# mumianyuxin/M3DSSD

Measured on AMD Instinct MI355X. Metric: images/sec at 1280x384 bs=8, 1/2/4/8 MI355X; 3D-box Linf vs ref, higher is better.
Workload: dtype f32; 1 GPU; BASELINE.json configs[1]: full M3d_inference_align (DLA-34 + DCNv2 align + ANAB) forward + decode + top-3000 + NMS, bs=8/GPU, 1280x384, fp32, random-init synthetic weights and frames; per_gpu_batch=8, global_batch=8, parallelism=dp1 (batch sharded, 1 all-gather of [B,40,14] detections)

## Files before the change

include/m3dssd_hip.h:

```cpp
#ifndef M3DSSD_HIP_H
#define M3DSSD_HIP_H

#include <stdint.h>

#ifdef __cplusplus
extern "C" {
#endif

typedef void *m3d_stream_t;

enum {
    M3D_OK = 0,
    M3D_E_ARG = -1,
    M3D_E_HIP = -2,
    M3D_E_WORKSPACE = -3
};

const char *m3d_last_error(void);
#define M3D_ABI_VERSION 5
int m3d_abi_version(void);
const char *m3d_source_hashes(void);

typedef struct m3d_conv_desc {
    const float *in;
// ... 263 lines not shown
    M3D_RPN_STAT_IOU_ACC = 7,
    M3D_RPN_STAT_ACC_FG = 8,
    M3D_RPN_STAT_ACC_BG = 9,
    M3D_RPN_STAT_N_FG = 10,
    M3D_RPN_STAT_N_BG = 11,
    M3D_RPN_STAT_FG_NUM = 12,
    M3D_RPN_STAT_BG_NUM = 13,
    M3D_RPN_STAT_N_ACTIVE = 14,
    M3D_RPN_STAT_FG_WEIGHT = 15,
    M3D_RPN_STAT_COUNT = 16
};
long long m3d_rpn_loss_workspace_bytes(int B, long long R);
int m3d_rpn_targets(const double *anchors, int A, int H, int W, const double *conf, int n_conf, const double *gt_table, int B,
                    int Gmax, const float *cls, const float *prob, int C, short *labels, short *gt_index, float *targets,
                    float *scores, void *workspace, long long workspace_bytes, m3d_stream_t stream);
int m3d_rpn_loss(const double *anchors, int A, int H, int W, const double *conf, int n_conf, const double *gt_table, int B,
                 int Gmax, const float *cls, const float *bbox_2d, const float *bbox_3d, int C, const short *labels,
                 const float *targets, const float *scores, unsigned char *sampled, float *grad_cls, float *grad_bbox_2d,
                 float *grad_bbox_3d, float *loss, double *stats, void *workspace, long long workspace_bytes,
                 m3d_stream_t stream);

enum {
    M3D_RPN_SMP_STAT_BAD_LABELS = 16,
    M3D_RPN_SMP_STAT_COUNT = 17
};
int m3d_rpn_precompute_targets(const double *anchors, int A, int H, int W, const double *conf, int n_conf,
                               const double *gt_table, int B, int Gmax, short *labels, short *gt_index, float *bbox_2d_tar,
                               float *bbox_3d_tar, int *any_val, void *workspace, long long workspace_bytes,
                               m3d_stream_t stream);
int m3d_rpn_loss_smp(const double *anchors, int A, int H, int W, const double *conf, int n_conf, int B, const void *labels_in,
                     int label_bytes, const float *bbox_2d_tar, const float *bbox_3d_tar, const int *any_val, const float *cls,
                     const float *prob, const float *bbox_2d, const float *bbox_3d, int C, short *labels, float *targets,
                     float *scores, unsigned char *sampled, float *grad_cls, float *grad_bbox_2d, float *grad_bbox_3d,
                     float *loss, double *stats, void *workspace, long long workspace_bytes, m3d_stream_t stream);

#define M3D_RPN_TARGET_STATS_COLS 23
long long m3d_rpn_target_stats_workspace_bytes(int B, long long R);
int m3d_rpn_target_stats(const double *anchors, int A, int H, int W, const double *conf, int n_conf, const double *gt_table, int B,
                         int Gmax, const double *center, double *out, void *workspace, long long workspace_bytes,
                         m3d_stream_t stream);

int m3d_pack_conv_weight(const float *w, float *packed, int Cout, int Cout_pad, int Cin, int Cin_pad, int kh,
                         int kw, m3d_stream_t stream);
int m3d_nchw_to_nhwc(const float *in, float *out, int N, int C, int H, int W, int out_cs, m3d_stream_t stream);
int m3d_nhwc_to_nchw(const float *in, int in_cs, float *out, int N, int C, int H, int W, m3d_stream_t stream);

int m3d_stem_conv7x7(const float *img_nchw, const float *wgt , const float *scale,
                     const float *shift, float *out, int out_cs, int N, int H, int W, m3d_stream_t stream);
int m3d_preprocess_u8(const unsigned char *frames_bgr, int N, int img_h, int img_w, const float *mean3, const float *stds3,
                      float *out_nchw, int H, int W, m3d_stream_t stream);
int m3d_stem_conv7x7_u8(const unsigned char *frames_bgr, int img_h, int img_w, const float *mean3, const float *stds3,
                        const float *wgt, const float *scale, const float *shift, float *out, int out_cs, int N, int H, int W,
                        m3d_stream_t stream);
#define M3D_AUGMENT_PARAMS 14
int m3d_augment_u8(const unsigned char *frames_bgr, int N, int hmax, int wmax, const double *params, int param_stride,
                   const float *mean3, const float *stds3, float *out_nchw, int H, int W, m3d_stream_t stream);
int m3d_conv3x3_c16(const float *in, int in_cs, const float *wgt, const float *scale, const float *shift, float *out,
                    int out_cs, int N, int H, int W, m3d_stream_t stream);
int m3d_conv3x3_c16_wino(const float *in, int in_cs, const float *U, const float *scale, const float *shift, float *out,
                         int out_cs, int N, int H, int W, m3d_stream_t stream);
int m3d_maxpool2x2(const float *in, int in_cs, float *out, int out_cs, int N, int H, int W, int C,
                   m3d_stream_t stream);
int m3d_upsample2x_add(const float *in, int in_cs, const float *wgt, const float *skip, int skip_cs,
                       float *out, int out_cs, int N, int H, int W, int C, m3d_stream_t stream);

int m3d_anchor_select(const float *cls_planar, int B, int A, int num_classes, int HW, int *sel_idx,
                      float *sel_prob, float *fg_all, m3d_stream_t stream);
int m3d_anchor_select_keys(const float *cls_planar, int B, int A, int HW, int *sel_idx, float *sel_prob,
                           unsigned int *score_bits, m3d_stream_t stream);
int m3d_fg_top1(const float *prob, int B, int A, int HW, int *idx, float *val, m3d_stream_t stream);
int m3d_align_offsets(int mode, const int *sel_idx, const float *sel_prob, float thresh, const float *table,
                      const float *bbox_x, const float *bbox_y, const float *anchor_wh, float mean_x,
                      float std_x, float mean_y, float std_y, float *offmask, int om_cs, int B, int A, int HW,
                      int kk, long long box_img_stride, m3d_stream_t stream);
int m3d_align_offsets_gated(const int *sel_idx, const float *sel_prob, float thresh, const float *bbox_x, const float *bbox_y,
                            const float *anchor_wh, float mean_x, float std_x, float mean_y, float std_y,
                            const unsigned char *need, float *offmask, int om_cs, int B, int A, int HW,
                            long long box_img_stride, m3d_stream_t stream);

int m3d_anab_pool_partial(const float *kv, int kv_cs, const float *s, int s_cs, const int *items, int n_items,
                          const int *bin_scale, int n_bins, float *partial, int max_slots, int B, int H, int W,
                          int C, m3d_stream_t stream);
int m3d_anab_pool_finish(const float *partial, const int *bin_slots, const float *bin_inv_area, int n_bins,
                         int max_slots, int Ck, int Cv, float *khat, int keys_pad, int ck_pad, float *vhatT,
                         int B, int frag, m3d_stream_t stream);
long long m3d_anab_pool_nested_scratch_bytes(int B, int C);
int m3d_anab_pool_nested(const float *kv, int kv_cs, const float *s, int s_cs, int B, int H, int W, int Ck, int Cv,
                         float *scratch, float *khat, int keys_pad, int ck_pad, float *vhatT, int frag, m3d_stream_t stream);
int m3d_anab_pool_nested_bf16(const void *kv, int kv_cs, const float *s, int s_cs, int B, int H, int W, int Ck, int Cv,
                              float *scratch, float *khat, int keys_pad, int ck_pad, float *vhatT, int frag, m3d_stream_t stream);
int m3d_anab_pool_nested_bf16_ex(const void *kv, int kv_cs, const float *s, int s_cs, int B, int H, int W, int Ck, int Cv,
                                 float *scratch, float *khat, int keys_pad, int ck_pad, float *vhatT, int frag,
                                 void *khat16, void *vhat16, m3d_stream_t stream);
int m3d_anab_attend_f32(const float *q, int q_cs, const float *khat, int k_cs, const float *vhatT, int B, int HW, int Ck,
                        int keys, int keys_pad, int Cv, const float *res, int res_cs, int res_mode, const float *scale,
                        const float *shift, int act, float *out, int out_cs, m3d_stream_t stream);
int m3d_anab_attend_f32_rows(const float *q, int q_cs, const float *khat, int k_cs, const float *vhatT, int B, int HW, int Ck,
                             int keys, int keys_pad, int Cv, const float *res, int res_cs, int res_mode, const float *scale,
                             const float *shift, int act, float *out, int out_cs, const int *rows, const int *n_rows,
                             m3d_stream_t stream);
long long m3d_anab_attention_workspace_bytes(int B, int H, int W, int Ck, int Cv, int backward);
int m3d_anab_attention_forward(const float *q, const float *k, const float *v, const float *g, float *out, int B, int H, int W, int Ck,
                               int Cv, int q_cs, int k_cs, int v_cs, int g_cs, int out_cs, void *workspace, long long workspace_bytes,
                               m3d_stream_t stream);
int m3d_anab_attention_backward(const float *q, const float *k, const float *v, const float *g, const float *grad_out, float *grad_q,
                                float *grad_k, float *grad_v, float *grad_g, int B, int H, int W, int Ck, int Cv, int q_cs, int k_cs,
// ... 83 lines not shown
```

m3dssd_amd/_hip.py:

```python
import ctypes
import os
import subprocess

_HERE = os.path.dirname(os.path.abspath(__file__))
CSRC = os.path.join(_HERE, "csrc")
SO_PATH = os.environ.get("M3D_HIP_LIB") or os.path.join(CSRC, "build", "libm3dssd_hip.so")
HEADER = os.path.join(os.path.dirname(_HERE), "include", "m3dssd_hip.h")

c_int, c_float, c_ll, c_void_p = ctypes.c_int, ctypes.c_float, ctypes.c_longlong, ctypes.c_void_p


class ConvDesc(ctypes.Structure):
    _fields_ = [
        ("inp", c_void_p), ("in_cs", c_int),
        ("N", c_int), ("H", c_int), ("W", c_int), ("Cin", c_int),
        ("wgt", c_void_p), ("wgt_img_stride", c_ll),
        ("Cout", c_int), ("Cout_pad", c_int),
        ("kh", c_int), ("kw", c_int), ("stride", c_int), ("pad", c_int), ("dil", c_int),
        ("Ho", c_int), ("Wo", c_int),
        ("out", c_void_p), ("out_cs", c_int), ("out_nchw", c_int), ("out_img_stride", c_ll),
        ("scale", c_void_p), ("shift", c_void_p),
        ("res", c_void_p), ("res_cs", c_int), ("res_mode", c_int),
        ("act", c_int), ("sigmoid_from", c_int),
        ("dcn_offmask", c_void_p), ("dcn_om_cs", c_int),
# ... 113 lines not shown
    "m3d_head_mlp_forward_batched": (c_int, [ctypes.POINTER(MlpDesc), c_int, P]),
    "m3d_head_mlp_forward_rows": (c_int, [ctypes.POINTER(MlpDesc), c_int, P, P, ctypes.c_uint, P]),
    "m3d_wino_conv3x3_forward": (c_int, [ctypes.POINTER(ConvDesc), P]),
    "m3d_wino_conv3x3_forward_ex": (c_int, [ctypes.POINTER(ConvDesc), c_int, P]),
    "m3d_wino_conv3x3_splitk_plan": (c_int, [ctypes.POINTER(ConvDesc), ctypes.POINTER(c_int), ctypes.POINTER(c_ll)]),
    "m3d_wino_conv3x3_variant": (c_int, [ctypes.POINTER(ConvDesc)]),
    "m3d_wino44_applicable": (c_int, [ctypes.POINTER(ConvDesc)]),
    "m3d_wino44_conv3x3_forward": (c_int, [ctypes.POINTER(ConvDesc), P]),
    "m3d_wino44_conv3x3_forward_ex": (c_int, [ctypes.POINTER(ConvDesc), c_int, P]),
    "m3d_wino44_kpair": (c_int, [ctypes.POINTER(ConvDesc)]),
    "m3d_wino44_conv3x3_forward_touch": (c_int, [ctypes.POINTER(ConvDesc), c_int, P, c_ll, P]),
    "m3d_cache_touch": (c_int, [P, c_ll, P]),
    "m3d_upload_indirect": (c_int, [P, P, c_ll, P]),
    "m3d_wino44_splitk_plan": (c_int, [ctypes.POINTER(ConvDesc), ctypes.POINTER(c_int), ctypes.POINTER(c_ll)]),
    "m3d_conv_wave_applicable": (c_int, [ctypes.POINTER(ConvDesc)]),
    "m3d_conv_wave_splitk_plan": (c_int, [ctypes.POINTER(ConvDesc), ctypes.POINTER(c_int), ctypes.POINTER(c_ll)]),
    "m3d_conv_wave_forward": (c_int, [ctypes.POINTER(ConvDesc), P]),
    "m3d_conv_wave_forward_wgsplit": (c_int, [ctypes.POINTER(ConvDesc), P]),
    "m3d_conv_wave_wgsplit_width": (c_int, [ctypes.POINTER(ConvDesc), ctypes.POINTER(c_int), ctypes.POINTER(c_int)]),
    "m3d_conv2d_tile": (c_int, [ctypes.POINTER(ConvDesc)] + [ctypes.POINTER(c_int)] * 4),
    "m3d_conv2d_splitk_plan": (c_int, [ctypes.POINTER(ConvDesc), ctypes.POINTER(c_int), ctypes.POINTER(c_ll)]),
    "m3d_dcn_v2_workspace_bytes": (c_ll, [c_int] * 10),
    "m3d_dcn_v2_workspace_bytes_grouped": (c_ll, [c_int] * 11),
    "m3d_dcn_v2_forward": (c_int, [P] * 6 + [c_int] * 14 + [P, c_ll, P]),
    "m3d_dcn_v2_backward_workspace_bytes": (c_ll, [c_int] * 11),
    "m3d_dcn_v2_backward": (c_int, [P] * 10 + [c_int] * 14 + [P, c_ll, P]),
    "m3d_dcn_v2_workspace_bytes_bf16": (c_ll, [c_int] * 11),
    "m3d_dcn_v2_forward_bf16": (c_int, [P, P, P, P, c_int, P, c_int, P] + [c_int] * 14 + [P, c_ll, P]),
    "m3d_dcn_v2_backward_workspace_bytes_bf16": (c_ll, [c_int] * 11),
    "m3d_dcn_v2_backward_bf16": (c_int, [P, P, P, c_int, P, c_int, P] + [P] * 5 + [c_int] * 14 + [P, c_ll, P]),
    "m3d_dcn_v2_psroi_pooling_workspace_bytes": (c_ll, [c_int] * 10),
    "m3d_dcn_v2_psroi_pooling_forward": (c_int, [P] * 5 + [c_int] * 8 + [c_float] + [c_int] * 5 + [c_float, P, c_ll, P]),
    "m3d_dcn_v2_psroi_pooling_backward": (c_int, [P] * 6 + [c_int] * 8 + [c_float] + [c_int] * 5 + [c_float, P, c_ll, P]),
    "m3d_rpn_loss_workspace_bytes": (c_ll, [c_int, c_ll]),
    "m3d_rpn_targets": (c_int, [P, c_int, c_int, c_int, P, c_int, P, c_int, c_int, P, P, c_int, P, P, P, P, P, c_ll, P]),
    "m3d_rpn_loss": (c_int, [P, c_int, c_int, c_int, P, c_int, P, c_int, c_int, P, P, P, c_int, P, P, P, P, P, P, P, P, P, P, c_ll, P]),
    "m3d_rpn_precompute_targets": (c_int, [P, c_int, c_int, c_int, P, c_int, P, c_int, c_int, P, P, P, P, P, P, c_ll, P]),
    "m3d_rpn_loss_smp": (c_int, [P, c_int, c_int, c_int, P, c_int, c_int, P, c_int, P, P, P, P, P, P, P, c_int] + [P] * 10 + [c_ll, P]),
    "m3d_rpn_target_stats_workspace_bytes": (c_ll, [c_int, c_ll]),
    "m3d_rpn_target_stats": (c_int, [P, c_int, c_int, c_int, P, c_int, P, c_int, c_int, P, P, P, c_ll, P]),
    "m3d_pack_conv_weight": (c_int, [P, P] + [c_int] * 6 + [P]),
    "m3d_nchw_to_nhwc": (c_int, [P, P] + [c_int] * 5 + [P]),
    "m3d_nhwc_to_nchw": (c_int, [P, c_int, P] + [c_int] * 4 + [P]),
    "m3d_stem_conv7x7": (c_int, [P, P, P, P, P] + [c_int] * 4 + [P]),
    "m3d_refine_3d": (c_int, [P, P, c_int, c_int, P, P, ctypes.c_double, c_int, ctypes.c_double, ctypes.c_double, P, P]),
    "m3d_refine_3d_ex": (c_int, [P, P, c_int, c_int, P, P, P, P, ctypes.c_double, c_int, ctypes.c_double, ctypes.c_double, P, P]),
    "m3d_refine_3d_host": (c_int, [P, P, c_int, c_int, P, P, P, P, ctypes.c_double, c_int, ctypes.c_double, ctypes.c_double, P]),
    "m3d_preprocess_u8": (c_int, [P, c_int, c_int, c_int, ctypes.POINTER(ctypes.c_float), ctypes.POINTER(ctypes.c_float), P, c_int,
                                  c_int, P]),
    "m3d_augment_u8": (c_int, [P, c_int, c_int, c_int, ctypes.POINTER(ctypes.c_double), c_int, ctypes.POINTER(ctypes.c_float),
                               ctypes.POINTER(ctypes.c_float), P, c_int, c_int, P]),
    "m3d_stem_conv7x7_u8": (c_int, [P, c_int, c_int, ctypes.POINTER(ctypes.c_float), ctypes.POINTER(ctypes.c_float), P, P, P, P,
                                    c_int, c_int, c_int, c_int, P]),
    "m3d_conv3x3_c16": (c_int, [P, c_int, P, P, P, P, c_int, c_int, c_int, c_int, P]),
    "m3d_conv3x3_c16_wino": (c_int, [P, c_int, P, P, P, P, c_int, c_int, c_int, c_int, P]),
    "m3d_maxpool2x2": (c_int, [P, c_int, P, c_int] + [c_int] * 4 + [P]),
    "m3d_upsample2x_add": (c_int, [P, c_int, P, P, c_int, P, c_int] + [c_int] * 4 + [P]),
    "m3d_anchor_select": (c_int, [P] + [c_int] * 4 + [P, P, P, P]),
    "m3d_anchor_select_keys": (c_int, [P] + [c_int] * 3 + [P, P, P, P]),
    "m3d_fg_top1": (c_int, [P, c_int, c_int, c_int, P, P, P]),
    "m3d_align_offsets": (c_int, [c_int, P, P, c_float, P, P, P, P] + [c_float] * 4 + [P] + [c_int] * 5 + [c_ll, P]),
    "m3d_align_offsets_gated": (c_int, [P, P, c_float, P, P, P] + [c_float] * 4 + [P, P] + [c_int] * 4 + [c_ll, P]),
    "m3d_anab_pool_partial": (c_int, [P, c_int, P, c_int, P, c_int, P, c_int, P] + [c_int] * 5 + [P]),
    "m3d_anab_pool_finish": (c_int, [P, P, P] + [c_int] * 4 + [P, c_int, c_int, P, c_int, c_int, P]),
    "m3d_anab_pool_nested_scratch_bytes": (c_ll, [c_int, c_int]),
    "m3d_anab_pool_nested": (c_int, [P, c_int, P, c_int, c_int, c_int, c_int, c_int, c_int, P, P, c_int, c_int, P, c_int, P]),
    "m3d_anab_attend_f32": (c_int, [P, c_int, P, c_int, P, c_int, c_int, c_int, c_int, c_int, c_int, P, c_int, c_int, P, P, c_int, P, c_int, P]),
    "m3d_anab_attend_f32_rows": (c_int, [P, c_int, P, c_int, P, c_int, c_int, c_int, c_int, c_int, c_int, P, c_int, c_int, P, P, c_int, P, c_int,
                                         P, P, P]),
    "m3d_anab_pool_nested_bf16": (c_int, [P, c_int, P, c_int, c_int, c_int, c_int, c_int, c_int, P, P, c_int, c_int, P, c_int, P]),
    "m3d_anab_pool_nested_bf16_ex": (c_int, [P, c_int, P, c_int, c_int, c_int, c_int, c_int, c_int, P, P, c_int, c_int, P, c_int, P, P, P]),
    "m3d_anab_attention_workspace_bytes": (c_ll, [c_int] * 6),
    "m3d_anab_attention_forward": (c_int, [P] * 5 + [c_int] * 10 + [P, c_ll, P]),
    "m3d_anab_attention_backward": (c_int, [P] * 9 + [c_int] * 14 + [P, c_ll, P]),
    "m3d_anab_attention_workspace_bytes_bf16": (c_ll, [c_int] * 6),
    "m3d_anab_attention_forward_bf16": (c_int, [P] * 5 + [c_int] * 10 + [P, c_ll, P]),
    "m3d_anab_attention_backward_bf16": (c_int, [P] * 9 + [c_int] * 14 + [P, c_ll, P]),
    "m3d_softmax_rows": (c_int, [P, c_int, c_int, c_int, P]),
    "m3d_bundle_outputs": (c_int, [P] * 7 + [c_int] * 3 + [P]),
    "m3d_decode_rows": (c_int, [P] * 9 + [c_int] * 3 + [P]),
    "m3d_topk_decode_workspace_bytes": (c_ll, [c_int, c_int]),
    "m3d_topk_decode": (c_int, [P] * 11 + [c_ll] + [c_int] * 3 + [P]),
    "m3d_topk_decode_scaled": (c_int, [P] * 12 + [c_ll] + [c_int] * 3 + [P]),
    "m3d_score_keys_planar": (c_int, [P, P, c_int, c_int, c_int, P]),
    "m3d_topk_decode_planar": (c_int, [P] * 11 + [c_ll] + [c_int] * 4 + [P]),
    "m3d_topk_decode_mw_workspace_bytes": (c_ll, [c_int, c_int, c_int]),
    "m3d_need_rows_workspace_bytes": (c_ll, [c_int, c_int]),
    "m3d_need_rows": (c_int, [P] + [c_int] * 4 + [P] * 5 + [c_ll, P]),
    "m3d_topk_decode_planar_mw": (c_int, [P] * 11 + [c_ll] + [c_int] * 5 + [P]),
    "m3d_select_post": (c_int, [P] * 3 + [c_int] * 3 + [P, P, P]),
    "m3d_nms_workspace_bytes": (c_ll, [c_int, c_int]),
    "m3d_nms_sorted_dev": (c_int, [P, c_int, c_int, c_int, c_float, P, P, P, P]),
    "_nms": (None, [P, P, P, c_int, c_int, c_float, c_int]),
    "m3d_rotate_iou_eval": (c_int, [P, c_int, P, c_int, c_int, P, P]),
    "m3d_eval_image_box_overlap": (c_int, [P, c_int, P, c_int, c_int, P]),
    "m3d_eval_d3_overlap": (c_int, [P, c_int, P, c_int, P, c_int]),
    "m3d_eval_statistics": (c_int, [P, c_ll, P, c_int, P, c_int, P, P, P, c_int, c_int, ctypes.c_double, ctypes.c_double,
                                    c_int, c_int, P, P, ctypes.POINTER(c_int)]),
    "m3d_eval_fused_statistics": (c_int, [P, c_ll, P, P, P, P, c_int, P, P, P, P, P, c_int, ctypes.c_double, P, c_int, c_int]),
    "m3d_clock_probe": (c_int, [P, ctypes.c_double, P]),
    "m3d_event_create": (c_int, [ctypes.POINTER(c_void_p)]),
    "m3d_event_record": (c_int, [P, P]),
    "m3d_event_elapsed_ms": (c_int, [P, P, ctypes.POINTER(c_float)]),
    "m3d_event_destroy": (c_int, [P]),
}

# ... 45 lines not shown
```

m3dssd_amd/csrc/backbone_kernels.hip:

```cpp

#include "common.h"

__global__ void pack_weight_kernel(const float *__restrict__ w, float *__restrict__ p, int Cout, int Cout_pad,
                                   int Cin, int Cin_pad, int KK, int Ctot, int c0)
{
    const long long total = (long long)Cout_pad * KK * Cin_pad;
    for (long long i = blockIdx.x * (long long)blockDim.x + threadIdx.x; i < total;
         i += (long long)gridDim.x * blockDim.x) {
        const int c = (int)(i % Cin_pad);
        const int tap = (int)((i / Cin_pad) % KK);
        const int co = (int)(i / ((long long)Cin_pad * KK));
        p[i] = (co < Cout && c < Cin) ? w[((long long)co * Ctot + c0 + c) * KK + tap] : 0.f;
    }
}

int m3d_pack_conv_weight_slice(const float *w, int Ctot, int c0, float *packed, int Cout, int Cout_pad, int Cin, int Cin_pad,
                               int kh, int kw, m3d_stream_t stream)
{
    M3D_REQUIRE(w && packed && Cout > 0 && Cout_pad >= Cout && Cin_pad >= Cin && c0 >= 0 && c0 + Cin <= Ctot,
                "pack_conv_weight: bad arguments");
    const long long total = (long long)Cout_pad * kh * kw * Cin_pad;
    hipLaunchKernelGGL(pack_weight_kernel, dim3(imin(cdiv(total, 256), 4096)), dim3(256), 0, (hipStream_t)stream, w,
                       packed, Cout, Cout_pad, Cin, Cin_pad, kh * kw, Ctot, c0);
    M3D_LAUNCH_CHECK();
// ... 19 lines not shown
    __syncthreads();
    for (int r = ty; r < 32; r += 8) {
        const int p = p0 + r, c = c0 + tx;
        if (c < C && p < HW) out[((size_t)n * HW + p) * out_cs + c] = t[tx][r];
    }
}

__global__ void nhwc_to_nchw_kernel(const float *__restrict__ in, int in_cs, float *__restrict__ out, int C, int HW)
{
    __shared__ float t[32][33];
    const int n = blockIdx.z, c0 = blockIdx.y * 32, p0 = blockIdx.x * 32;
    const int tx = threadIdx.x & 31, ty = threadIdx.x >> 5;
    for (int r = ty; r < 32; r += 8) {
        const int p = p0 + r, c = c0 + tx;
        t[r][tx] = (c < C && p < HW) ? in[((size_t)n * HW + p) * in_cs + c] : 0.f;
    }
    __syncthreads();
    for (int r = ty; r < 32; r += 8) {
        const int c = c0 + r, p = p0 + tx;
        if (c < C && p < HW) out[((size_t)n * C + c) * HW + p] = t[tx][r];
    }
}

int m3d_nchw_to_nhwc_slice(const float *in, int Ctot, int c0, float *out, int N, int C, int H, int W, int out_cs,
                           m3d_stream_t stream)
{
    M3D_REQUIRE(in && out && out_cs >= C && c0 >= 0 && c0 + C <= Ctot, "nchw_to_nhwc: bad arguments");
    const int HW = H * W;
    hipLaunchKernelGGL(nchw_to_nhwc_kernel, dim3(cdiv(HW, 32), cdiv(C, 32), N), dim3(256), 0, (hipStream_t)stream, in,
                       out, C, HW, out_cs, Ctot, c0);
    M3D_LAUNCH_CHECK();
    return M3D_OK;
}

extern "C" int m3d_nchw_to_nhwc(const float *in, float *out, int N, int C, int H, int W, int out_cs,
                                m3d_stream_t stream)
{
    return m3d_nchw_to_nhwc_slice(in, C, 0, out, N, C, H, W, out_cs, stream);
}

extern "C" int m3d_nhwc_to_nchw(const float *in, int in_cs, float *out, int N, int C, int H, int W,
                                m3d_stream_t stream)
{
    M3D_REQUIRE(in && out && in_cs >= C, "nhwc_to_nchw: bad arguments");
    const int HW = H * W;
    hipLaunchKernelGGL(nhwc_to_nchw_kernel, dim3(cdiv(HW, 32), cdiv(C, 32), N), dim3(256), 0, (hipStream_t)stream, in,
                       in_cs, out, C, HW);
    M3D_LAUNCH_CHECK();
    return M3D_OK;
}

#define STEM_TH 8
#define STEM_TW 32
struct U8Norm {
    float mean[3], stds[3];
    int img_h, img_w;
};
__device__ __forceinline__ float u8_normalise(const unsigned char *__restrict__ frame, const U8Norm &nm, int h, int w, int c_rgb)
{
    const int cb = 2 - c_rgb;
    float v = (h < nm.img_h && w < nm.img_w) ? (float)frame[((size_t)h * nm.img_w + w) * 3 + cb] : 0.f;
    v = v / 255.0f;
    v = v - nm.mean[cb];
    return v / nm.stds[cb];
}

template <bool U8>
__global__ __launch_bounds__(256) void stem_conv7x7_kernel(const void *__restrict__ img_, const float *__restrict__ wgt,
                                                           const float *__restrict__ scale,
                                                           const float *__restrict__ shift, float *__restrict__ out,
                                                           int out_cs, int H, int W, U8Norm nm)
{
    const float *img = static_cast<const float *>(img_);
    constexpr int PH = STEM_TH + 6, PW = STEM_TW + 6;
    __shared__ float patch[3][PH][PW + 1];
    const int n = blockIdx.z, h0 = blockIdx.y * STEM_TH, w0 = blockIdx.x * STEM_TW;
    const float *im = img + (size_t)n * 3 * H * W;
    const unsigned char *frame = static_cast<const unsigned char *>(img_) + (size_t)n * nm.img_h * nm.img_w * 3;
    {
        constexpr int NE = 3 * PH * PW, NIT = (NE + 255) / 256;
        float v[NIT];
#pragma unroll
        for (int k = 0; k < NIT; ++k) {
            const int i = threadIdx.x + 256 * k;
            const int c = i / (PH * PW), r = (i / PW) % PH, q = i % PW;
            const int h = h0 + r - 3, w = w0 + q - 3;
            const bool inside = i < NE && h >= 0 && h < H && w >= 0 && w < W;
            if constexpr (U8) v[k] = inside ? u8_normalise(frame, nm, h, w, c) : 0.f;
            else v[k] = inside ? im[((size_t)c * H + h) * W + w] : 0.f;
        }
#pragma unroll
        for (int k = 0; k < NIT; ++k) {
            const int i = threadIdx.x + 256 * k;
            if (i < NE) patch[i / (PH * PW)][(i / PW) % PH][i % PW] = v[k];
        }
    }
    __syncthreads();
    const int ty = threadIdx.x / STEM_TW, tx = threadIdx.x % STEM_TW;
    f32x2 acc2[8];
#pragma unroll
    for (int o = 0; o < 8; ++o) acc2[o] = f32x2{0.f, 0.f};
    for (int i = 0; i < 7; ++i) {
#pragma unroll
        for (int j = 0; j < 7; ++j) {
#pragma unroll
            for (int c = 0; c < 3; ++c) {
                const float v = patch[c][ty + i][tx + j];
                const f32x2 vv = {v, v};
                const float *wp = wgt + ((i * 7 + j) * 3 + c) * 16;
#pragma unroll
                for (int o = 0; o < 8; ++o) acc2[o] = __builtin_elementwise_fma(vv, f32x2{wp[2 * o], wp[2 * o + 1]}, acc2[o]);
            }
        }
    }
    float acc[16];
#pragma unroll
    for (int o = 0; o < 8; ++o) { acc[2 * o] = acc2[o][0]; acc[2 * o + 1] = acc2[o][1]; }
    const int h = h0 + ty, w = w0 + tx;
    if (h < H && w < W) {
        float *op = out + ((size_t)(n * H + h) * W + w) * out_cs;
#pragma unroll
        for (int o4 = 0; o4 < 4; ++o4) {
            f32x4 v;
#pragma unroll
            for (int e = 0; e < 4; ++e) v[e] = leaky(acc[o4 * 4 + e] * scale[o4 * 4 + e] + shift[o4 * 4 + e]);
            *reinterpret_cast<f32x4 *>(op + o4 * 4) = v;
        }
    }
}

extern "C" int m3d_stem_conv7x7(const float *img_nchw, const float *wgt, const float *scale, const float *shift,
                                float *out, int out_cs, int N, int H, int W, m3d_stream_t stream)
{
    M3D_REQUIRE(img_nchw && wgt && scale && shift && out && out_cs % 4 == 0 && out_cs >= 16, "stem: bad arguments");
    hipLaunchKernelGGL(stem_conv7x7_kernel<false>, dim3(cdiv(W, STEM_TW), cdiv(H, STEM_TH), N), dim3(256), 0,
                       (hipStream_t)stream, (const void *)img_nchw, wgt, scale, shift, out, out_cs, H, W, U8Norm{});
    M3D_LAUNCH_CHECK();
    return M3D_OK;
}

static int fill_u8norm(U8Norm &nm, const float *mean3, const float *stds3, int img_h, int img_w, int H, int W)
{
    M3D_REQUIRE(mean3 && stds3, "preprocess: mean / stds are host pointers to 3 floats each");
    M3D_REQUIRE(img_h >= 1 && img_w >= 1 && img_h <= H && img_w <= W,
                "preprocess: the frame (%dx%d) must fit the padded size (%dx%d)", img_h, img_w, H, W);
    for (int c = 0; c < 3; ++c) {
        M3D_REQUIRE(stds3[c] != 0.f, "preprocess: zero std");
        nm.mean[c] = mean3[c];
        nm.stds[c] = stds3[c];
    }
    nm.img_h = img_h; nm.img_w = img_w;
    return M3D_OK;
}

extern "C" int m3d_stem_conv7x7_u8(const unsigned char *frames_bgr, int img_h, int img_w, const float *mean3, const float *stds3,
                                   const float *wgt, const float *scale, const float *shift, float *out, int out_cs, int N, int H,
                                   int W, m3d_stream_t stream)
{
    M3D_REQUIRE(frames_bgr && wgt && scale && shift && out && out_cs % 4 == 0 && out_cs >= 16, "stem_u8: bad arguments");
    U8Norm nm;
    const int rc = fill_u8norm(nm, mean3, stds3, img_h, img_w, H, W);
    if (rc != M3D_OK) return rc;
    hipLaunchKernelGGL(stem_conv7x7_kernel<true>, dim3(cdiv(W, STEM_TW), cdiv(H, STEM_TH), N), dim3(256), 0,
                       (hipStream_t)stream, (const void *)frames_bgr, wgt, scale, shift, out, out_cs, H, W, nm);
    M3D_LAUNCH_CHECK();
    return M3D_OK;
}

__global__ void preprocess_u8_kernel(const unsigned char *__restrict__ frames, float *__restrict__ out, int N, int H, int W,
                                     U8Norm nm)
{
    const long long total = (long long)N * H * W;
    for (long long i = blockIdx.x * (long long)blockDim.x + threadIdx.x; i < total; i += (long long)gridDim.x * blockDim.x) {
        const int w = (int)(i % W);
        const long long t = i / W;
        const int h = (int)(t % H), n = (int)(t / H);
        const unsigned char *frame = frames + (size_t)n * nm.img_h * nm.img_w * 3;
#pragma unroll
        for (int c = 0; c < 3; ++c) out[(((size_t)n * 3 + c) * H + h) * W + w] = u8_normalise(frame, nm, h, w, c);
    }
}

extern "C" int m3d_preprocess_u8(const unsigned char *frames_bgr, int N, int img_h, int img_w, const float *mean3,
                                 const float *stds3, float *out_nchw, int H, int W, m3d_stream_t stream)
{
    M3D_REQUIRE(frames_bgr && out_nchw && N >= 1, "preprocess_u8: bad arguments");
    U8Norm nm;
    const int rc = fill_u8norm(nm, mean3, stds3, img_h, img_w, H, W);
    if (rc != M3D_OK) return rc;
    const long long total = (long long)N * H * W;
    hipLaunchKernelGGL(preprocess_u8_kernel, dim3(imin(cdiv(total, 256), 16384)), dim3(256), 0, (hipStream_t)stream, frames_bgr,
                       out_nchw, N, H, W, nm);
    M3D_LAUNCH_CHECK();
    return M3D_OK;
}

#define L0_TH 8
#define L0_TW 32
#define L0_PS 20
__global__ __launch_bounds__(256) void conv3x3_c16_kernel(const float *__restrict__ in, int in_cs,
                                                          const float *__restrict__ wgt, const float *__restrict__ scale,
                                                          const float *__restrict__ shift, float *__restrict__ out,
                                                          int out_cs, int H, int W)
{
    constexpr int PH = L0_TH + 2, PW = L0_TW + 2;
    __shared__ __attribute__((aligned(16))) float tile[PH * PW * L0_PS];
    const int n = blockIdx.z, h0 = blockIdx.y * L0_TH, w0 = blockIdx.x * L0_TW;
    for (int i = threadIdx.x; i < PH * PW * 4; i += 256) {
        const int q = i & 3, p = i >> 2;
        const int r = p / PW, c = p - r * PW;
        const int h = h0 + r - 1, w = w0 + c - 1;
        f32x4 v = {0.f, 0.f, 0.f, 0.f};
        if (h >= 0 && h < H && w >= 0 && w < W)
            v = *reinterpret_cast<const f32x4 *>(in + ((size_t)(n * H + h) * W + w) * in_cs + q * 4);
        *reinterpret_cast<f32x4 *>(tile + p * L0_PS + q * 4) = v;
    }
    __syncthreads();
    const int ty = threadIdx.x / L0_TW, tx = threadIdx.x % L0_TW;
    f32x2 acc2[8];
// ... 275 lines not shown
```

m3dssd_amd/engine.py:

```python
import ctypes
import math
import os

import numpy as np
import torch

from . import _hip
from ._hip import ConvDesc, MlpDesc
from .config import model_flags

BN_EPS = 1e-5
SELECT_KEYS = os.environ.get("M3D_SELECT_KEYS", "1") != "0"
SPARSE_HEADS_MAX_FRACTION = 0.5
PSP_SIZES = (1, 4, 8, 16)
BACKBONE_CHANNELS = {"dla34": (16, 32, 64, 128, 256, 512), "dla102": (16, 32, 128, 256, 512, 1024)}
DLA102_LEVELS = (1, 1, 1, 3, 4, 1)


def _rup(a, b):
    return (a + b - 1) // b * b


class View:
    __slots__ = ("t", "ptr", "n", "h", "w", "c", "cs", "keep")
# ... 67 lines not shown
    w = weight2d.detach().to(device, torch.float32)
    r, k = w.shape
    assert k % 8 == 0 and rows_pad % 32 == 0 and rows_pad >= r
    if rows_pad != r:
        w = torch.cat([w, w.new_zeros(rows_pad - r, k)], 0)
    return w.view(rows_pad // 32, 32, k // 8, 2, 4).permute(0, 2, 3, 1, 4).contiguous().view(-1)


_WINO_G = torch.tensor([[1.0, 0.0, 0.0], [0.5, 0.5, 0.5], [0.5, -0.5, 0.5], [0.0, 0.0, 1.0]], dtype=torch.float64)


def pack_wino(weight, cout_pad, device):
    g = weight.detach().to("cpu", torch.float64)
    co, ci = g.shape[0], g.shape[1]
    assert g.shape[2:] == (3, 3) and ci % 8 == 0 and cout_pad % 32 == 0 and cout_pad >= co
    u = torch.einsum("ai,ocij,bj->aboc", _WINO_G, g, _WINO_G).reshape(16, co, ci)
    if cout_pad != co:
        u = torch.cat([u, u.new_zeros(16, cout_pad - co, ci)], 1)
    u = u.view(16, cout_pad // 32, 32, ci // 8, 2, 4).permute(0, 1, 3, 4, 2, 5).contiguous()
    return u.to(torch.float32).reshape(-1).to(device)


_WINO44_G = torch.tensor([[1 / 4, 0, 0], [-1 / 6, -1 / 6, -1 / 6], [-1 / 6, 1 / 6, -1 / 6], [1 / 24, 1 / 12, 1 / 6], [1 / 24, -1 / 12, 1 / 6],
                          [0, 0, 1]], dtype=torch.float64)


def pack_wino44(weight, cout_pad, device):
    g = weight.detach().to("cpu", torch.float64)
    co, ci = g.shape[0], g.shape[1]
    assert g.shape[2:] == (3, 3) and ci % 16 == 0 and cout_pad % 32 == 0 and cout_pad >= co
    u = torch.einsum("ai,ocij,bj->aboc", _WINO44_G, g, _WINO44_G).reshape(36, co, ci)
    if cout_pad != co:
        u = torch.cat([u, u.new_zeros(36, cout_pad - co, ci)], 1)
    u = u.view(36, cout_pad // 32, 2, 16, ci // 16, 4, 4).permute(1, 4, 0, 2, 5, 3, 6).contiguous()
    return u.to(torch.float32).reshape(-1).to(device)


def pack_wino44_c16(weight, device):
    g = weight.detach().to("cpu", torch.float64)
    assert tuple(g.shape) == (16, 16, 3, 3)
    u = torch.einsum("ai,ocij,bj->abco", _WINO44_G, g, _WINO44_G).reshape(36, 4, 4, 16)
    return u.permute(0, 1, 3, 2).contiguous().to(torch.float32).reshape(-1).to(device)


WINO_MIN_BLOCKS = int(os.environ.get("M3D_WINO_MIN_BLOCKS", "128"))
FUSED_ANAB = os.environ.get("M3D_FUSED_ANAB", "1") != "0"
ANAB_ROWS = os.environ.get("M3D_ANAB_ROWS", "1") != "0"
USE_ANAB_WAVE = os.environ.get("M3D_ANAB_WAVE", "1") != "0"
USE_ANAB_NESTED = os.environ.get("M3D_ANAB_NESTED", "1") != "0"
USE_DCN_WAVE = os.environ.get("M3D_DCN_WAVE", "1") != "0"
USE_CONV_WAVE = os.environ.get("M3D_CONV_WAVE", "1") != "0"
USE_CONV_WAVE_WGSPLIT = os.environ.get("M3D_CONV_WAVE_WGSPLIT", "1") != "0"
USE_OFFMASK_WAVE = os.environ.get("M3D_OFFMASK_WAVE", "1") != "0"
USE_WINO = os.environ.get("M3D_WINO", "1") != "0"
USE_WINO44 = os.environ.get("M3D_WINO44", "1") != "0"
WINO44_TOUCH = os.environ.get("M3D_WINO44_TOUCH", "1") != "0"
WINO44_TOUCH_SPAN = int(os.environ.get("M3D_WINO44_TOUCH_SPAN", "2"))
USE_WINO44_SPLITK = os.environ.get("M3D_WINO44_SPLITK", "1") != "0"
W44_SPLIT_NB = 2 if os.environ.get("M3D_W44_SPLIT_NB", "1") == "2" else 1
W44_SPLIT_KPAIR = os.environ.get("M3D_W44_SPLIT_NB", "1") == "3"
WINO44_MIN_WGS = int(os.environ.get("M3D_WINO44_MIN_WGS", "1000000"))
WINO44_MIN_WGS_NB1 = int(os.environ.get("M3D_WINO44_MIN_WGS_NB1", "200"))


class OpCost:

    def __init__(self, hbm_bytes):
        self.hbm_bytes = int(hbm_bytes)


def lo_hi_contains(start, end, n, br):
    lo, hi = start, (n if end is None else end)
    return lo <= br[0] and br[2] <= hi


class _Plan:

    def __init__(self):
        self.ops = []
        self.keep = []
        self.named = {}
        self.w44_prev = None
        self.branches = []
        self.tail = None
        self.tail_start = None


class Engine:
    def __init__(self, state_dict, conf, device=None, backbone_only=False):
        self.L = _hip.lib()
        self.backbone_only = backbone_only
        self.device = torch.device(device if device is not None else conf.device)
        if self.device.type != "cuda":
            raise NotImplementedError("the M3DSSD HIP engine runs on a ROCm device only (got %s)" % self.device)
        if self.device.index is None:
            self.device = torch.device("cuda", torch.cuda.current_device())
        self.conf = conf
        self.back_bone = str(conf.back_bone) if "back_bone" in conf else "dla34"
        if self.back_bone not in BACKBONE_CHANNELS:
            raise NotImplementedError("back_bone %r: the engine runs %s" % (self.back_bone, " / ".join(BACKBONE_CHANNELS)))
        if getattr(self, "compute_dtype", "f32") == "bf16" and self.back_bone != "dla34":
            raise NotImplementedError("the bf16 engine runs the dla34 backbone only; run back_bone %r in fp32" % self.back_bone)
        sd = {k[7:] if k.startswith("module.") else k: v for k, v in state_dict.items()}
        self.sd = sd
        self.A = int(np.asarray(conf.anchors).shape[0]) if not backbone_only else 0
        self.NC = len(conf.lbls) + 1 if not backbone_only else 0
# ... 247 lines not shown
            if wsplits.value > 1 and USE_CONV_WAVE_WGSPLIT and (d.Cout_pad % 64 == 0 or (USE_OFFMASK_WAVE and wsplits.value <= 4)):
                frag = pc.frag()
                d.wgt = frag.data_ptr()
                kind = "conv_wave<%s>" % ",".join((["deform"] if om is not None else []) + ["wgsplit%d" % wsplits.value])
                plan.ops.append((name, kind, flops_true, lambda st: _hip.check(L.m3d_conv_wave_forward_wgsplit(ref, st)), d))
                return
            ws = None
            if wsplits.value > 1 and wbytes.value > 0:
                ws = torch.empty(wbytes.value // 4, device=self.device, dtype=torch.float32)
                d.splitk_ws, d.splitk_ws_bytes = ws.data_ptr(), wbytes.value
            if L.m3d_conv_wave_applicable(ref) > 0:
                frag = pc.frag()
                d.wgt = frag.data_ptr()
                if ws is not None:
                    plan.keep.append(ws)
                kind = "conv_wave%s" % ("<%s>" % ",".join(
                    (["deform"] if om is not None else []) + (["splitk%d" % wsplits.value] if wsplits.value > 1 else []))
                    if (om is not None or wsplits.value > 1) else "")
                plan.ops.append((name, kind, flops_true, lambda st: _hip.check(L.m3d_conv_wave_forward(ref, st)), d))
                return
            d.splitk_ws, d.splitk_ws_bytes = None, 0
        bm, bn, bk, grid = ctypes.c_int(), ctypes.c_int(), ctypes.c_int(), ctypes.c_int()
        _hip.check(L.m3d_conv2d_tile(ref, ctypes.byref(bm), ctypes.byref(bn), ctypes.byref(bk), ctypes.byref(grid)))
        splits, ws_bytes = ctypes.c_int(), ctypes.c_longlong()
        _hip.check(L.m3d_conv2d_splitk_plan(ref, ctypes.byref(splits), ctypes.byref(ws_bytes)))
        if splits.value > 1:
            ws = torch.empty(ws_bytes.value // 4, device=self.device, dtype=torch.float32)
            plan.keep.append(ws)
            d.splitk_ws, d.splitk_ws_bytes = ws.data_ptr(), ws_bytes.value
        kind = "igemm<%d,%d,%d%s%s%s>" % (bm.value, bn.value, bk.value, ",deform" if om is not None else "",
                                          ",planar" if planar is not None else "",
                                          ",splitk%d" % splits.value if splits.value > 1 else "")
        if cin_true is None:
            cin_true = pc.cin if (pc is not None and wgt_ptr is None) else x.c
        flops = 2.0 * x.n * d.Ho * d.Wo * d.Cout * kh * kw * cin_true
        plan.ops.append((name, kind, flops, lambda st: _hip.check(L.m3d_conv2d_forward(ref, st)), d))

    def _op(self, plan, name, kind, fn, flops=0.0, nbytes=None):
        plan.ops.append((name, kind, float(flops), fn, OpCost(nbytes) if nbytes is not None else None))

    def _build_plan(self, B, H, W):
        L, P = self.L, self.P
        plan = _Plan()
        chs = BACKBONE_CHANNELS[self.back_bone]
        b = "base.base"
        in_ptr = [0]
        plan.named["input_ptr"] = in_ptr
        s0 = self._buf(plan, B, H, W, 16)
        in_u8 = [0, 0, 0]
        plan.named["input_u8"] = in_u8
        mean3 = (ctypes.c_float * 3)(*[float(v) for v in self.conf.image_means])
        stds3 = (ctypes.c_float * 3)(*[float(v) for v in self.conf.image_stds])

        def stem(st):
            if in_u8[0]:
                _hip.check(L.m3d_stem_conv7x7_u8(in_u8[0], in_u8[1], in_u8[2], mean3, stds3, P["stem.w"].data_ptr(),
                                                 P["stem.scale"].data_ptr(), P["stem.shift"].data_ptr(), s0.ptr, s0.cs, B, H,
                                                 W, st))
            else:
                _hip.check(L.m3d_stem_conv7x7(in_ptr[0], P["stem.w"].data_ptr(), P["stem.scale"].data_ptr(),
                                              P["stem.shift"].data_ptr(), s0.ptr, s0.cs, B, H, W, st))
        self._op(plan, "stem", "stem", stem, flops=2.0 * B * H * W * 16 * 147, nbytes=B * H * W * (3 + 16) * 4)
        l0 = self._buf(plan, B, H, W, 16, name="level0")
        if P.get("level0.wino44") is not None and H % 4 == 0 and W % 4 == 0 and os.environ.get("M3D_LEVEL0_WINO44", "1") != "0":
            pc0 = P["level0"]
            self._op(plan, "level0", "wino44_c16", lambda st: _hip.check(L.m3d_conv3x3_c16_wino(
                s0.ptr, s0.cs, P["level0.wino44"].data_ptr(), pc0.scale.data_ptr(), pc0.shift.data_ptr(), l0.ptr, l0.cs,
                B, H, W, st)), flops=2.0 * B * H * W * 16 * 144, nbytes=B * H * W * 32 * 4)
        elif P["level0.direct"] is not None and os.environ.get("M3D_LEVEL0_IGEMM", "0") != "1":
            pc0 = P["level0"]
            self._op(plan, "level0", "conv3x3_c16", lambda st: _hip.check(L.m3d_conv3x3_c16(
                s0.ptr, s0.cs, P["level0.direct"].data_ptr(), pc0.scale.data_ptr(), pc0.shift.data_ptr(), l0.ptr, l0.cs,
                B, H, W, st)), flops=2.0 * B * H * W * 16 * 144, nbytes=B * H * W * 32 * 4)
        else:
            self._conv(plan, "level0", P["level0"], s0, l0, 1, 1, act=1)
        l1 = self._buf(plan, B, H // 2, W // 2, 32, name="level1")
        self._conv(plan, "level1", P["level1"], l0, l1, 2, 1, act=1)

        def maxpool(name, x, out):
            self._op(plan, name, "maxpool", lambda st: _hip.check(L.m3d_maxpool2x2(
                x.ptr, x.cs, out.ptr, out.cs, x.n, x.h, x.w, x.c, st)), nbytes=x.n * x.h * x.w * x.c * 5)

        if self.back_bone == "dla102":
            l3, l4, l5 = self._dla102_levels(plan, l1, maxpool)
        else:
            def block(p, x, res, out, stride):
                co = P[p + ".conv1"].cout
                t = self._buf(plan, B, out.h, out.w, co)
                self._conv(plan, p + ".conv1", P[p + ".conv1"], x, t, stride, 1, act=1)
                self._conv(plan, p + ".conv2", P[p + ".conv2"], t, out, 1, 1, act=1, res=res)

            def tree1(p, x, co, stride, out, bottom=None):
                h, w = x.h // stride, x.w // stride
                cat = self._buf(plan, B, h, w, 2 * co)
                x2v, x1v = cat.slice(0, co), cat.slice(co, co)
                if stride == 1:
                    bottom = x
                elif bottom is None:
                    bottom = self._buf(plan, B, h, w, x.c)
                    maxpool(p + ".downsample", x, bottom)
                if (p + ".project") in P:
                    res = self._buf(plan, B, h, w, co)
                    self._conv(plan, p + ".project", P[p + ".project"], bottom, res, 1, 0, act=0)
                else:
                    res = bottom
                block(p + ".tree1", x, res, x1v, stride)
                block(p + ".tree2", x1v, x1v, x2v, 1)
                self._conv(plan, p + ".root", P[p + ".root"], cat, out, 1, 0, act=1)

            l2 = self._buf(plan, B, H // 4, W // 4, 64, name="level2")
            tree1(b + ".level2", l1, 64, 2, l2)

            def tree2(p, x, co, out):
                ci = x.c
# ... 539 lines not shown
```

Measured before the change: 1570 images/sec.

## Add MFMA-based persistent stem 7x7 conv with prefetched input tiles

Adds a new stem 7x7 conv kernel that computes the 147-tap reduction with 16x16x4 f32 MFMA instructions. Each workgroup walks a run of tiles and prefetches the next tile's input rows into registers while computing the current one. It is enabled by default through M3D_STEM_MFMA=1 (form 1 uses 15 tiles per workgroup), with the old scalar kernel kept as the fallback for form 0. The aim is to cut the stem's FMA-bound time and hide input load latency, at the cost of register pressure under tight launch bounds and a zero-padded K layout.

```diff
diff --git a/include/m3dssd_hip.h b/include/m3dssd_hip.h
--- a/include/m3dssd_hip.h
+++ b/include/m3dssd_hip.h
@@ -339,6 +339,11 @@
 int m3d_stem_conv7x7_u8(const unsigned char *frames_bgr, int img_h, int img_w, const float *mean3, const float *stds3,
                         const float *wgt, const float *scale, const float *shift, float *out, int out_cs, int N, int H, int W,
                         m3d_stream_t stream);
+int m3d_stem_conv7x7_form(const float *img_nchw, const float *wgt , const float *scale, const float *shift,
+                          float *out, int out_cs, int N, int H, int W, int form, m3d_stream_t stream);
+int m3d_stem_conv7x7_u8_form(const unsigned char *frames_bgr, int img_h, int img_w, const float *mean3, const float *stds3,
+                             const float *wgt, const float *scale, const float *shift, float *out, int out_cs, int N, int H,
+                             int W, int form, m3d_stream_t stream);
 #define M3D_AUGMENT_PARAMS 14
 int m3d_augment_u8(const unsigned char *frames_bgr, int N, int hmax, int wmax, const double *params, int param_stride,
                    const float *mean3, const float *stds3, float *out_nchw, int H, int W, m3d_stream_t stream);
diff --git a/m3dssd_amd/_hip.py b/m3dssd_amd/_hip.py
--- a/m3dssd_amd/_hip.py
+++ b/m3dssd_amd/_hip.py
@@ -189,6 +189,9 @@
                                ctypes.POINTER(ctypes.c_float), P, c_int, c_int, P]),
     "m3d_stem_conv7x7_u8": (c_int, [P, c_int, c_int, ctypes.POINTER(ctypes.c_float), ctypes.POINTER(ctypes.c_float), P, P, P, P,
                                     c_int, c_int, c_int, c_int, P]),
+    "m3d_stem_conv7x7_form": (c_int, [P, P, P, P, P] + [c_int] * 5 + [P]),
+    "m3d_stem_conv7x7_u8_form": (c_int, [P, c_int, c_int, ctypes.POINTER(ctypes.c_float), ctypes.POINTER(ctypes.c_float), P, P, P, P,
+                                         c_int, c_int, c_int, c_int, c_int, P]),
     "m3d_conv3x3_c16": (c_int, [P, c_int, P, P, P, P, c_int, c_int, c_int, c_int, P]),
     "m3d_conv3x3_c16_wino": (c_int, [P, c_int, P, P, P, P, c_int, c_int, c_int, c_int, P]),
     "m3d_maxpool2x2": (c_int, [P, c_int, P, c_int] + [c_int] * 4 + [P]),
diff --git a/m3dssd_amd/csrc/backbone_kernels.hip b/m3dssd_amd/csrc/backbone_kernels.hip
--- a/m3dssd_amd/csrc/backbone_kernels.hip
+++ b/m3dssd_amd/csrc/backbone_kernels.hip
@@ -95,17 +95,22 @@
 
 #define STEM_TH 8
 #define STEM_TW 32
+__device__ __forceinline__ float stem_epi(float acc, float sc, float sh) { return leaky(acc * sc + sh); }
 struct U8Norm {
     float mean[3], stds[3];
     int img_h, img_w;
 };
+__device__ __forceinline__ float u8_norm_value(float v, float mean, float stds)
+{
+    v = v / 255.0f;
+    v = v - mean;
+    return v / stds;
+}
 __device__ __forceinline__ float u8_normalise(const unsigned char *__restrict__ frame, const U8Norm &nm, int h, int w, int c_rgb)
 {
     const int cb = 2 - c_rgb;
-    float v = (h < nm.img_h && w < nm.img_w) ? (float)frame[((size_t)h * nm.img_w + w) * 3 + cb] : 0.f;
-    v = v / 255.0f;
-    v = v - nm.mean[cb];
-    return v / nm.stds[cb];
+    const float v = (h < nm.img_h && w < nm.img_w) ? (float)frame[((size_t)h * nm.img_w + w) * 3 + cb] : 0.f;
+    return u8_norm_value(v, nm.mean[cb], nm.stds[cb]);
 }
 
 template <bool U8>
@@ -166,20 +171,169 @@
         for (int o4 = 0; o4 < 4; ++o4) {
             f32x4 v;
 #pragma unroll
-            for (int e = 0; e < 4; ++e) v[e] = leaky(acc[o4 * 4 + e] * scale[o4 * 4 + e] + shift[o4 * 4 + e]);
+            for (int e = 0; e < 4; ++e) v[e] = stem_epi(acc[o4 * 4 + e], scale[o4 * 4 + e], shift[o4 * 4 + e]);
             *reinterpret_cast<f32x4 *>(op + o4 * 4) = v;
         }
     }
+}
+
+#define STEMM_WGS_PER_CU(u8) ((u8) ? 3 : 4)
+#define STEMM_TILES_PER_WG 15
+struct StemWalk {
+    int tiles_x, tiles_y, ntiles, grid;
+    int per_wg;
+};
+template <bool U8>
+__global__ __launch_bounds__(256, STEMM_WGS_PER_CU(U8)) void stem_conv7x7_mfma_kernel(const void *__restrict__ img_, const float *__restrict__ wgt,
+                                                                const float *__restrict__ scale,
+                                                                const float *__restrict__ shift, float *__restrict__ out,
+                                                                int out_cs, int H, int W, U8Norm nm, StemWalk wk)
+{
+    constexpr int PH = STEM_TH + 6, PW = STEM_TW + 6, D = 3 * PW - 21;
+    constexpr int NP = 3 * PH, NIT = (NP + 3) / 4;
+    __shared__ float smem[4 + PH * PW * 3];
+    float *const patch = smem + 4;
+    if (threadIdx.x < 4) smem[threadIdx.x] = 0.f;
+    const int tid = threadIdx.x, lane = tid & 63, wave = __builtin_amdgcn_readfirstlane(tid >> 6);
+    const int li = lane & 15, lq = lane >> 4;
+    float wf[37];
+#pragma unroll
+    for (int s = 0; s < 37; ++s) {
+        const int k = 4 * s + lq - 1;
+        const float w = wgt[(k < 0 ? 0 : k) * 16 + li];
+        wf[s] = (s > 0 || k >= 0) ? w : 0.f;
+    }
+    float sc[4], sh[4];
+#pragma unroll
+    for (int e = 0; e < 4; ++e) { sc[e] = scale[4 * lq + e]; sh[e] = shift[4 * lq + e]; }
+    const unsigned oobv = M3D_BUF_OOB;
+    const unsigned out_lane = (unsigned)(li * out_cs + 4 * lq) * 4u;
+    const unsigned img_bytes = U8 ? (unsigned)(nm.img_h * nm.img_w * 3) : (unsigned)(3 * H * W) * 4u;
+
+    const int tile0 = blockIdx.x * wk.per_wg, tile_end = min(tile0 + wk.per_wg, wk.ntiles);
+    int tx, ty, n;
+    {
+        const int t0 = tile0, t1 = t0 / wk.tiles_x;
+        tx = t0 - t1 * wk.tiles_x;
+        n = t1 / wk.tiles_y;
+        ty = t1 - n * wk.tiles_y;
+    }
+    float v[NIT];
+    bool col_in = false;
+    auto request = [&](int n_, int ty_, int tx_) {
+        const int h0 = ty_ * STEM_TH, wcol = tx_ * STEM_TW + lane - 3;
+        col_in = lane < PW && wcol >= 0 && wcol < W;
+        const char *base = static_cast<const char *>(img_) + (size_t)n_ * img_bytes;
+        const __amdgpu_buffer_rsrc_t rimg = make_rsrc(base, img_bytes);
+        const unsigned voff = U8 ? ((col_in && wcol < nm.img_w) ? (unsigned)wcol * 3u : oobv) : (col_in ? (unsigned)wcol * 4u : oobv);
+#pragma unroll
+        for (int it = 0; it < NIT; ++it) {
+            const int p = wave + 4 * it, c = p / PH, r = p - c * PH, h = h0 + r - 3;
+            if constexpr (U8) {
+                const bool row_ok = p < NP && h >= 0 && h < nm.img_h;
+                const unsigned soff = row_ok ? (unsigned)(h * nm.img_w) * 3u + (unsigned)(2 - c) : 0u;
+                v[it] = (float)__builtin_amdgcn_raw_buffer_load_b8(rimg, row_ok ? voff : oobv, soff, 0);
+            } else {
+                const bool row_ok = p < NP && h >= 0 && h < H;
+                const unsigned soff = row_ok ? (unsigned)((c * H + h) * W) * 4u : 0u;
+                v[it] = __builtin_bit_cast(float, __builtin_amdgcn_raw_buffer_load_b32(rimg, row_ok ? voff : oobv, soff, 0));
+            }
+        }
+    };
+    request(n, ty, tx);
+    for (int tile = tile0; tile < tile_end; ++tile) {
+        const int h0 = ty * STEM_TH, w0 = tx * STEM_TW, n0 = n;
+#pragma unroll
+        for (int it = 0; it < NIT; ++it) {
+            const int p = wave + 4 * it, c = p / PH, r = p - c * PH;
+            float x = v[it];
+            if constexpr (U8) {
+                const int cb = 2 - c, h = h0 + r - 3;
+                const float mean = cb == 0 ? nm.mean[0] : cb == 1 ? nm.mean[1] : nm.mean[2];
+                const float stds = cb == 0 ? nm.stds[0] : cb == 1 ? nm.stds[1] : nm.stds[2];
+                x = (col_in && h >= 0 && h < H) ? u8_norm_value(x, mean, stds) : 0.f;
+            }
+            if (p < NP && lane < PW) patch[(r * PW + lane) * 3 + c] = x;
+        }
+        __syncthreads();
+        if (++tx == wk.tiles_x) { tx = 0; ++ty; }
+        if (ty == wk.tiles_y) { ty = 0; ++n; }
+        if (tile + 1 < tile_end) request(n, ty, tx);
+        const float *pb[4];
+        pb[0] = patch + ((2 * wave) * PW + li) * 3 + lq;
+#pragma unroll
+        for (int t = 1; t < 4; ++t) pb[t] = pb[0] + (lq >= t ? D : 0);
+        f32x4 acc[2][2];
+#pragma unroll
+        for (int rr = 0; rr < 2; ++rr)
+#pragma unroll
+            for (int ct = 0; ct < 2; ++ct) acc[rr][ct] = f32x4{0.f, 0.f, 0.f, 0.f};
+#pragma unroll
+        for (int s = 0; s < 37; ++s) {
+            const int kb = 4 * s - 1, r0 = kb < 0 ? 0 : kb / 21;
+            const int t = (kb + 1) / 21 > r0 ? 1 : (kb + 2) / 21 > r0 ? 2 : (kb + 3) / 21 > r0 ? 3 : 0;
+            float a[2][2];
+#pragma unroll
+            for (int rr = 0; rr < 2; ++rr)
+#pragma unroll
+                for (int ct = 0; ct < 2; ++ct) a[rr][ct] = pb[t][kb + r0 * D + (rr * PW + ct * 16) * 3];
+#pragma unroll
+            for (int rr = 0; rr < 2; ++rr)
+#pragma unroll
+                for (int ct = 0; ct < 2; ++ct)
+                    acc[rr][ct] = __builtin_amdgcn_mfma_f32_16x16x4f32(wf[s], a[rr][ct], acc[rr][ct], 0, 0, 0);
+        }
+        const int rows = min(STEM_TH, H - h0);
+        const __amdgpu_buffer_rsrc_t rout = make_rsrc(out + (size_t)(n0 * H + h0) * W * out_cs, (unsigned)(rows * W * out_cs) * 4u);
+#pragma unroll
+        for (int ct = 0; ct < 2; ++ct) {
+            const unsigned vo = (w0 + ct * 16 + li < W) ? out_lane : oobv;
+#pragma unroll
+            for (int rr = 0; rr < 2; ++rr) {
+                f32x4 o;
+#pragma unroll
+                for (int e = 0; e < 4; ++e) o[e] = stem_epi(acc[rr][ct][e], sc[e], sh[e]);
+                if (2 * wave + rr < rows)
+                    buf_store_f32x4_nop(o, rout, vo, (unsigned)(((2 * wave + rr) * W + w0 + ct * 16) * out_cs) * 4u);
+            }
+        }
+        __syncthreads();
+    }
+}
+
+static bool stem_use_mfma(int form) { return form != 0; }
+
+static bool stem_walk(StemWalk &wk, int N, int H, int W, int out_cs, long long img_bytes, int form)
+{
+    const long long tiles = (long long)cdiv(W, STEM_TW) * cdiv(H, STEM_TH) * N;
+    if (img_bytes >= (1ll << 31) || (long long)STEM_TH * W * out_cs * 4 >= (1ll << 31) || tiles >= (1ll << 30) || (long long)W * H * 12 >= (1ll << 31))
+        return false;
+    wk.tiles_x = cdiv(W, STEM_TW); wk.tiles_y = cdiv(H, STEM_TH); wk.ntiles = (int)tiles;
+    wk.per_wg = form >= 2 ? form : STEMM_TILES_PER_WG;
+    wk.grid = cdiv(tiles, wk.per_wg);
+    return true;
+}
+
+extern "C" int m3d_stem_conv7x7_form(const float *img_nchw, const float *wgt, const float *scale, const float *shift,
+                                     float *out, int out_cs, int N, int H, int W, int form, m3d_stream_t stream)
+{
+    M3D_REQUIRE(img_nchw && wgt && scale && shift && out && out_cs % 4 == 0 && out_cs >= 16, "stem: bad arguments");
+    const dim3 grid(cdiv(W, STEM_TW), cdiv(H, STEM_TH), N);
+    StemWalk wk;
+    if (stem_use_mfma(form) && stem_walk(wk, N, H, W, out_cs, 12ll * H * W, form))
+        hipLaunchKernelGGL(stem_conv7x7_mfma_kernel<false>, dim3(wk.grid), dim3(256), 0, (hipStream_t)stream, (const void *)img_nchw,
+                           wgt, scale, shift, out, out_cs, H, W, U8Norm{}, wk);
+    else
+        hipLaunchKernelGGL(stem_conv7x7_kernel<false>, grid, dim3(256), 0, (hipStream_t)stream, (const void *)img_nchw, wgt,
+                           scale, shift, out, out_cs, H, W, U8Norm{});
+    M3D_LAUNCH_CHECK();
+    return M3D_OK;
 }
 
 extern "C" int m3d_stem_conv7x7(const float *img_nchw, const float *wgt, const float *scale, const float *shift,
                                 float *out, int out_cs, int N, int H, int W, m3d_stream_t stream)
 {
-    M3D_REQUIRE(img_nchw && wgt && scale && shift && out && out_cs % 4 == 0 && out_cs >= 16, "stem: bad arguments");
-    hipLaunchKernelGGL(stem_conv7x7_kernel<false>, dim3(cdiv(W, STEM_TW), cdiv(H, STEM_TH), N), dim3(256), 0,
-                       (hipStream_t)stream, (const void *)img_nchw, wgt, scale, shift, out, out_cs, H, W, U8Norm{});
-    M3D_LAUNCH_CHECK();
-    return M3D_OK;
+    return m3d_stem_conv7x7_form(img_nchw, wgt, scale, shift, out, out_cs, N, H, W, -1, stream);
 }
 
 static int fill_u8norm(U8Norm &nm, const float *mean3, const float *stds3, int img_h, int img_w, int H, int W)
@@ -196,18 +350,31 @@
     return M3D_OK;
 }
 
-extern "C" int m3d_stem_conv7x7_u8(const unsigned char *frames_bgr, int img_h, int img_w, const float *mean3, const float *stds3,
-                                   const float *wgt, const float *scale, const float *shift, float *out, int out_cs, int N, int H,
-                                   int W, m3d_stream_t stream)
+extern "C" int m3d_stem_conv7x7_u8_form(const unsigned char *frames_bgr, int img_h, int img_w, const float *mean3,
+                                        const float *stds3, const float *wgt, const float *scale, const float *shift, float *out,
+                                        int out_cs, int N, int H, int W, int form, m3d_stream_t stream)
 {
     M3D_REQUIRE(frames_bgr && wgt && scale && shift && out && out_cs % 4 == 0 && out_cs >= 16, "stem_u8: bad arguments");
     U8Norm nm;
     const int rc = fill_u8norm(nm, mean3, stds3, img_h, img_w, H, W);
     if (rc != M3D_OK) return rc;
-    hipLaunchKernelGGL(stem_conv7x7_kernel<true>, dim3(cdiv(W, STEM_TW), cdiv(H, STEM_TH), N), dim3(256), 0,
-                       (hipStream_t)stream, (const void *)frames_bgr, wgt, scale, shift, out, out_cs, H, W, nm);
-    M3D_LAUNCH_CHECK();
-    return M3D_OK;
+    const dim3 grid(cdiv(W, STEM_TW), cdiv(H, STEM_TH), N);
+    StemWalk wk;
+    if (stem_use_mfma(form) && stem_walk(wk, N, H, W, out_cs, 3ll * img_h * img_w, form))
+        hipLaunchKernelGGL(stem_conv7x7_mfma_kernel<true>, dim3(wk.grid), dim3(256), 0, (hipStream_t)stream, (const void *)frames_bgr,
+                           wgt, scale, shift, out, out_cs, H, W, nm, wk);
+    else
+        hipLaunchKernelGGL(stem_conv7x7_kernel<true>, grid, dim3(256), 0, (hipStream_t)stream, (const void *)frames_bgr, wgt,
+                           scale, shift, out, out_cs, H, W, nm);
+    M3D_LAUNCH_CHECK();
+    return M3D_OK;
+}
+
+extern "C" int m3d_stem_conv7x7_u8(const unsigned char *frames_bgr, int img_h, int img_w, const float *mean3, const float *stds3,
+                                   const float *wgt, const float *scale, const float *shift, float *out, int out_cs, int N, int H,
+                                   int W, m3d_stream_t stream)
+{
+    return m3d_stem_conv7x7_u8_form(frames_bgr, img_h, img_w, mean3, stds3, wgt, scale, shift, out, out_cs, N, H, W, -1, stream);
 }
 
 __global__ void preprocess_u8_kernel(const unsigned char *__restrict__ frames, float *__restrict__ out, int N, int H, int W,
diff --git a/m3dssd_amd/engine.py b/m3dssd_amd/engine.py
--- a/m3dssd_amd/engine.py
+++ b/m3dssd_amd/engine.py
@@ -143,6 +143,7 @@
 USE_CONV_WAVE = os.environ.get("M3D_CONV_WAVE", "1") != "0"
 USE_CONV_WAVE_WGSPLIT = os.environ.get("M3D_CONV_WAVE_WGSPLIT", "1") != "0"
 USE_OFFMASK_WAVE = os.environ.get("M3D_OFFMASK_WAVE", "1") != "0"
+STEM_FORM = max(0, int(os.environ.get("M3D_STEM_MFMA", "1")))
 USE_WINO = os.environ.get("M3D_WINO", "1") != "0"
 USE_WINO44 = os.environ.get("M3D_WINO44", "1") != "0"
 WINO44_TOUCH = os.environ.get("M3D_WINO44_TOUCH", "1") != "0"
@@ -496,14 +497,16 @@
         mean3 = (ctypes.c_float * 3)(*[float(v) for v in self.conf.image_means])
         stds3 = (ctypes.c_float * 3)(*[float(v) for v in self.conf.image_stds])
 
+        stem_form = STEM_FORM
+
         def stem(st):
             if in_u8[0]:
-                _hip.check(L.m3d_stem_conv7x7_u8(in_u8[0], in_u8[1], in_u8[2], mean3, stds3, P["stem.w"].data_ptr(),
-                                                 P["stem.scale"].data_ptr(), P["stem.shift"].data_ptr(), s0.ptr, s0.cs, B, H,
-                                                 W, st))
+                _hip.check(L.m3d_stem_conv7x7_u8_form(in_u8[0], in_u8[1], in_u8[2], mean3, stds3, P["stem.w"].data_ptr(),
+                                                      P["stem.scale"].data_ptr(), P["stem.shift"].data_ptr(), s0.ptr, s0.cs, B, H,
+                                                      W, stem_form, st))
             else:
-                _hip.check(L.m3d_stem_conv7x7(in_ptr[0], P["stem.w"].data_ptr(), P["stem.scale"].data_ptr(),
-                                              P["stem.shift"].data_ptr(), s0.ptr, s0.cs, B, H, W, st))
+                _hip.check(L.m3d_stem_conv7x7_form(in_ptr[0], P["stem.w"].data_ptr(), P["stem.scale"].data_ptr(),
+                                                   P["stem.shift"].data_ptr(), s0.ptr, s0.cs, B, H, W, stem_form, st))
         self._op(plan, "stem", "stem", stem, flops=2.0 * B * H * W * 16 * 147, nbytes=B * H * W * (3 + 16) * 4)
         l0 = self._buf(plan, B, H, W, 16, name="level0")
         if P.get("level0.wino44") is not None and H % 4 == 0 and W % 4 == 0 and os.environ.get("M3D_LEVEL0_WINO44", "1") != "0":
```

Result: no change. 1565 images/sec (-0.3%).
